# csyxwei/FFWM

Hardware: AMD Instinct MI355X
Metric: train img/s (128x128, full FFWM GAN step) (higher is better)
Workload: dtype f32; 1 GPU; BASELINE configs[2]: full FFWM train step (netG+netD+flowNetF+flowNetB, all losses, 3x Adam), synthetic MultiPIE-shaped 128x128; batch_per_gpu=8, global_batch=8, parallelism=dp1, grad_buckets=10, bucket_MiB=64

## Files before the change

### ffwm_amd/csrc/conv_winograd_gemm.hip

```cpp
#include "common.hpp"

namespace ffwm {
namespace {

typedef float f32x16 __attribute__((ext_vector_type(16)));
typedef float f32x4 __attribute__((ext_vector_type(4)));

enum { kWgNone = FFWM_WG_NONE, kWgBias = FFWM_WG_BIAS, kWgBiasRelu = FFWM_WG_BIAS_RELU, kWgBiasMfm = FFWM_WG_BIAS_MFM };
constexpr int kWgStage = 16;

struct WgGeo {
    int C, C4;
    int H, W, K;
    int TH, TW, T;
    int Tp, Kp;
};

__device__ __forceinline__ float wg_max_nan(float a, float b) { return __builtin_isunordered(a, b) ? a + b : fmaxf(a, b); }
__device__ __forceinline__ float wg_relu_nan(float v) { return v != v ? v : fmaxf(v, 0.f); }

__global__ void __launch_bounds__(kBlock)
wg_weights_kernel(const float* __restrict__ w, float* __restrict__ U, int K, int C, int Cp, int mode) {
    const int64_t e = static_cast<int64_t>(blockIdx.x) * kBlock + threadIdx.x;
    if (e >= static_cast<int64_t>(K) * Cp) return;
    const int k = static_cast<int>(e / Cp), c = static_cast<int>(e - static_cast<int64_t>(k) * Cp);
    float g[3][3];
#pragma unroll
    for (int r = 0; r < 3; ++r)
#pragma unroll
        for (int s = 0; s < 3; ++s) {
            float v = 0.f;
            if (c < C) v = mode == 0 ? w[(static_cast<size_t>(k) * C + c) * 9 + r * 3 + s]
                                     : w[(static_cast<size_t>(c) * K + k) * 9 + (2 - r) * 3 + (2 - s)];
            g[r][s] = v;
        }
    float t[4][3];
#pragma unroll
    for (int s = 0; s < 3; ++s) {
        t[0][s] = g[0][s];
        t[1][s] = 0.5f * (g[0][s] + g[1][s] + g[2][s]);
        t[2][s] = 0.5f * (g[0][s] - g[1][s] + g[2][s]);
        t[3][s] = g[2][s];
    }
    const size_t pstride = static_cast<size_t>(Cp / 4) * K * 4;
    float* dst = U + (static_cast<size_t>(c >> 2) * K + k) * 4 + (c & 3);
#pragma unroll
    for (int i = 0; i < 4; ++i) {
        dst[(i * 4 + 0) * pstride] = t[i][0];
        dst[(i * 4 + 1) * pstride] = 0.5f * (t[i][0] + t[i][1] + t[i][2]);
        dst[(i * 4 + 2) * pstride] = 0.5f * (t[i][0] - t[i][1] + t[i][2]);
        dst[(i * 4 + 3) * pstride] = t[i][2];
    }
}

__global__ void __launch_bounds__(kBlock)
wg_input_transform_kernel(const float* __restrict__ x, const float* __restrict__ mask, float* __restrict__ V, const WgGeo g) {
    const int t = blockIdx.x * kBlock + threadIdx.x;
    if (t >= g.Tp) return;
    const int c4 = blockIdx.y;
    const bool tv = t < g.T;
    const int per = g.TH * g.TW;
    const int b = tv ? t / per : 0;
    const int rem = tv ? t - b * per : 0;
    const int ty = rem / g.TW, tx = rem - ty * g.TW;
    const size_t HW = static_cast<size_t>(g.H) * g.W;
    f32x4 v[16];
#pragma unroll
    for (int j = 0; j < 4; ++j) {
        const int c = c4 * 4 + j;
        const bool cv = tv && c < g.C;
        const size_t plane = (static_cast<size_t>(b) * g.C + (cv ? c : 0)) * HW;
        float d[16];
#pragma unroll
        for (int i = 0; i < 4; ++i)
#pragma unroll
            for (int q = 0; q < 4; ++q) {
                const int iy = 2 * ty - 1 + i, ix = 2 * tx - 1 + q;
                float e = 0.f;
                if (cv && iy >= 0 && iy < g.H && ix >= 0 && ix < g.W) {
                    const size_t o = plane + static_cast<size_t>(iy) * g.W + ix;
                    e = x[o];
                    if (mask != nullptr) e = mask[o] <= 0.f ? 0.f : e;
                }
                d[i * 4 + q] = e;
            }
#pragma unroll
        for (int i = 0; i < 4; ++i) {
            float r[4];
#pragma unroll
            for (int q = 0; q < 4; ++q)
                r[q] = i == 0 ? d[0 + q] - d[8 + q] : i == 1 ? d[4 + q] + d[8 + q] : i == 2 ? d[8 + q] - d[4 + q] : d[4 + q] - d[12 + q];
            v[i * 4 + 0][j] = r[0] - r[2];
            v[i * 4 + 1][j] = r[1] + r[2];
            v[i * 4 + 2][j] = r[2] - r[1];
            v[i * 4 + 3][j] = r[1] - r[3];
        }
    }
    const size_t pstride = static_cast<size_t>(g.C4) * g.Tp;
    f32x4* dst = reinterpret_cast<f32x4*>(V) + static_cast<size_t>(c4) * g.Tp + t;
#pragma unroll
    for (int p = 0; p < 16; ++p) dst[p * pstride] = v[p];
}

template <int TILE>
__global__ void __launch_bounds__(kBlock)
wg_batched_gemm_kernel(const float* __restrict__ U, const float* __restrict__ V, float* __restrict__ M, int K, int C4, int Tp, int Kp,
                       int KT, int TTn) {
    constexpr int WT = TILE / 2, NB = WT / 32, NL = TILE / 64;
    __shared__ f32x4 As[2][4][TILE];
    __shared__ f32x4 Bs[2][4][TILE];
    const int lane = threadIdx.x & 63, wave = threadIdx.x >> 6;
    const int l31 = lane & 31, half = lane >> 5;
    const int wm = wave >> 1, wn = wave & 1;
    unsigned bid = blockIdx.x;
    const int tt = static_cast<int>(bid % static_cast<unsigned>(TTn));
    bid /= static_cast<unsigned>(TTn);
    const int kt = static_cast<int>(bid % static_cast<unsigned>(KT));
    const int p = static_cast<int>(bid / static_cast<unsigned>(KT));
    const int k0 = kt * TILE, t0 = tt * TILE;
    const f32x4* Up = reinterpret_cast<const f32x4*>(U) + static_cast<size_t>(p) * C4 * K;
    const f32x4* Vp = reinterpret_cast<const f32x4*>(V) + static_cast<size_t>(p) * C4 * Tp;

    f32x4 ra[NL], rb[NL];
    auto gload = [&](int stage) {
#pragma unroll
        for (int i = 0; i < NL; ++i) {
            const int idx = threadIdx.x + kBlock * i;
            const int grp = stage * 4 + idx / TILE, n = idx % TILE;
            f32x4 a = {0.f, 0.f, 0.f, 0.f};
            if (k0 + n < K) a = Up[static_cast<size_t>(grp) * K + k0 + n];
            ra[i] = a;
            rb[i] = Vp[static_cast<size_t>(grp) * Tp + t0 + n];
        }
    };
    auto sstore = [&](int buf) {
#pragma unroll
        for (int i = 0; i < NL; ++i) {
            const int idx = threadIdx.x + kBlock * i;
            As[buf][idx / TILE][idx % TILE] = ra[i];
            Bs[buf][idx / TILE][idx % TILE] = rb[i];
        }
    };

    f32x16 acc[NB][NB];
#pragma unroll
    for (int i = 0; i < NB; ++i)
#pragma unroll
        for (int j = 0; j < NB; ++j)
#pragma unroll
            for (int r = 0; r < 16; ++r) acc[i][j][r] = 0.f;

    const int stages = C4 / 4;
    gload(0);
    sstore(0);
    __syncthreads();
    int buf = 0;
    for (int st = 0; st < stages; ++st) {
        const bool more = st + 1 < stages;
        if (more) gload(st + 1);
#pragma unroll
        for (int s = 0; s < 2; ++s) {
            f32x4 a[NB], b[NB];
#pragma unroll
            for (int i = 0; i < NB; ++i) {
                a[i] = As[buf][2 * s + half][wm * WT + i * 32 + l31];
                b[i] = Bs[buf][2 * s + half][wn * WT + i * 32 + l31];
            }
#pragma unroll
            for (int q = 0; q < 4; ++q)
#pragma unroll
                for (int i = 0; i < NB; ++i)
#pragma unroll
                    for (int j = 0; j < NB; ++j)
                        acc[i][j] = __builtin_amdgcn_mfma_f32_32x32x2f32(a[i][q], b[j][q], acc[i][j], 0, 0, 0);
        }
        if (more) sstore(buf ^ 1);
        __syncthreads();
        buf ^= 1;
    }

    float* Mp = M + (static_cast<size_t>(p) * Kp + k0 + wm * WT) * Tp + t0 + wn * WT + l31;
#pragma unroll
    for (int i = 0; i < NB; ++i)
#pragma unroll
        for (int j = 0; j < NB; ++j)
#pragma unroll
            for (int r = 0; r < 16; ++r) {
                const int row = i * 32 + (r & 3) + 8 * (r >> 2) + 4 * half;
                Mp[static_cast<size_t>(row) * Tp + j * 32] = acc[i][j][r];
            }
}

__device__ __forceinline__ void wg_tile_of(const float* __restrict__ M, size_t pstride, float bv, float (&y)[4]) {
    float z[4][2];
#pragma unroll
    for (int i = 0; i < 4; ++i) {
        const float m0 = M[(i * 4 + 0) * pstride], m1 = M[(i * 4 + 1) * pstride], m2 = M[(i * 4 + 2) * pstride], m3 = M[(i * 4 + 3) * pstride];
        z[i][0] = (m0 + m1) + m2;
        z[i][1] = (m1 - m2) - m3;
    }
#pragma unroll
    for (int j = 0; j < 2; ++j) {
        y[j] = ((z[0][j] + z[1][j]) + z[2][j]) + bv;
        y[2 + j] = ((z[1][j] - z[2][j]) - z[3][j]) + bv;
    }
}

__global__ void __launch_bounds__(kBlock)
wg_output_transform_kernel(const float* __restrict__ M, const float* __restrict__ bias, float* __restrict__ out, const WgGeo g, int epi,
                           int vec) {
    const int t = blockIdx.x * kBlock + threadIdx.x;
    if (t >= g.T) return;
    const int ko = blockIdx.y;
    const int Kout = epi == kWgBiasMfm ? g.K / 2 : g.K;
    const size_t pstride = static_cast<size_t>(g.Kp) * g.Tp;
    const bool use_bias = bias != nullptr && epi != kWgNone;
    float y[4];
    wg_tile_of(M + static_cast<size_t>(ko) * g.Tp + t, pstride, use_bias ? bias[ko] : 0.f, y);
    if (epi == kWgBiasRelu) {
#pragma unroll
        for (int v = 0; v < 4; ++v) y[v] = wg_relu_nan(y[v]);
    } else if (epi == kWgBiasMfm) {
        float y2[4];
        wg_tile_of(M + static_cast<size_t>(ko + Kout) * g.Tp + t, pstride, use_bias ? bias[ko + Kout] : 0.f, y2);
#pragma unroll
        for (int v = 0; v < 4; ++v) y[v] = wg_max_nan(y[v], y2[v]);
    }
    const int per = g.TH * g.TW;
    const int b = t / per, rem = t - b * per;
    const int ty = rem / g.TW, tx = rem - ty * g.TW;
    const int oy = 2 * ty, ox = 2 * tx;
    const bool row1 = oy + 1 < g.H, col1 = ox + 1 < g.W;
    float* o = out + ((static_cast<size_t>(b) * Kout + ko) * g.H + oy) * g.W + ox;
    if (vec) {
        *reinterpret_cast<float2*>(o) = make_float2(y[0], y[1]);
        if (row1) *reinterpret_cast<float2*>(o + g.W) = make_float2(y[2], y[3]);
    } else {
        o[0] = y[0];
        if (col1) o[1] = y[1];
        if (row1) {
            o[g.W] = y[2];
            if (col1) o[g.W + 1] = y[3];
        }
    }
}

}
}

using namespace ffwm;

static int64_t wg_round_up(int64_t v, int64_t m) { return (v + m - 1) / m * m; }

struct WgPlan {
    int tile;
    int64_t T, Tp, Kp, Cp;
    int64_t KT, TTn;
    int64_t v_floats, m_floats;
};
static WgPlan wg_plan(int64_t B, int64_t C, int64_t H, int64_t W, int64_t K, int force_tile) {
    WgPlan p;
    p.T = B * ((H + 1) / 2) * ((W + 1) / 2);
    p.Cp = wg_round_up(C, kWgStage);
    const int64_t n128 = 16 * ((K + 127) / 128) * ((p.T + 127) / 128);
    p.tile = force_tile ? force_tile : (n128 >= device_cus() ? 128 : 64);
    p.Tp = wg_round_up(p.T, p.tile);
    p.Kp = wg_round_up(K, p.tile);
    p.KT = p.Kp / p.tile;
    p.TTn = p.Tp / p.tile;
    p.v_floats = 16 * p.Cp * p.Tp;
    p.m_floats = 16 * p.Kp * p.Tp;
    return p;
}

extern "C" int64_t ffwm_conv3x3_wg_weights_bytes(int64_t K, int64_t C) {
    if (K <= 0 || C <= 0) return 0;
    return 16 * wg_round_up(C, kWgStage) * K * 4;
}

extern "C" int64_t ffwm_conv3x3_wg_workspace_bytes(int64_t B, int64_t C, int64_t H, int64_t W, int64_t K) {
    if (B <= 0 || C <= 0 || H <= 0 || W <= 0 || K <= 0) return 0;
    const int64_t T = wg_round_up(B * ((H + 1) / 2) * ((W + 1) / 2), 128);
    return 16 * T * (wg_round_up(C, kWgStage) + wg_round_up(K, 128)) * 4;
}

extern "C" int ffwm_conv3x3_wg_weights(const void* weight, void* U, int64_t K, int64_t C, int data_gradient, int dtype, void* stream) {
    const char* fn = "ffwm_conv3x3_wg_weights";
    FFWM_REQUIRE(dtype == FFWM_F32, FFWM_ERR_DTYPE, "%s: float32 only", fn);
    FFWM_REQUIRE(weight && U, FFWM_ERR_ARG, "%s: NULL tensor pointer", fn);
    FFWM_REQUIRE(K > 0 && C > 0, FFWM_ERR_ARG, "%s: sizes must be positive", fn);
    FFWM_REQUIRE(data_gradient == 0 || data_gradient == 1, FFWM_ERR_ARG, "%s: data_gradient must be 0 or 1", fn);
    const int64_t Cp = wg_round_up(C, kWgStage);
    FFWM_REQUIRE(K * Cp < (1LL << 31) - kBlock && K * C * 9 < (1LL << 31), FFWM_ERR_SIZE, "%s: weight beyond 2^31 elements", fn);
    hipStream_t st = static_cast<hipStream_t>(stream);
    LaunchScope ls("conv_wg_weights", st, 4.0 * (9.0 * K * C + 16.0 * K * Cp));
    hipLaunchKernelGGL(wg_weights_kernel, dim3(static_cast<unsigned>((K * Cp + kBlock - 1) / kBlock)), dim3(kBlock), 0, st,
                       static_cast<const float*>(weight), static_cast<float*>(U), static_cast<int>(K), static_cast<int>(C),
                       static_cast<int>(Cp), data_gradient);
    return check_launch(fn);
}

extern "C" int ffwm_conv3x3_wg_tile(int64_t B, int64_t C, int64_t H, int64_t W, int64_t K) {
    if (B <= 0 || C <= 0 || H <= 0 || W <= 0 || K <= 0) return 0;
    return wg_plan(B, C, H, W, K, 0).tile;
}

extern "C" int ffwm_conv3x3_wg_forward(const void* input, const void* U, const void* bias, void* output, void* workspace,
                                       int64_t B, int64_t C, int64_t H, int64_t W, int64_t K, int epilogue, const void* relu_mask,
                                       int dtype, void* stream) {
    return ffwm_conv3x3_wg_forward_tiled(input, U, bias, output, workspace, B, C, H, W, K, epilogue, relu_mask, 0, dtype, stream);
}

extern "C" int ffwm_conv3x3_wg_forward_tiled(const void* input, const void* U, const void* bias, void* output, void* workspace,
                                             int64_t B, int64_t C, int64_t H, int64_t W, int64_t K, int epilogue, const void* relu_mask,
                                             int tile, int dtype, void* stream) {
    const char* fn = "ffwm_conv3x3_wg_forward";
    FFWM_REQUIRE(dtype == FFWM_F32, FFWM_ERR_DTYPE, "%s: float32 only", fn);
    FFWM_REQUIRE(input && U && output && workspace, FFWM_ERR_ARG, "%s: NULL tensor pointer", fn);
    FFWM_REQUIRE(B > 0 && C > 0 && H > 0 && W > 0 && K > 0, FFWM_ERR_ARG, "%s: sizes must be positive", fn);
    const int epi = epilogue;
    FFWM_REQUIRE(epi >= kWgNone && epi <= kWgBiasMfm, FFWM_ERR_ARG,
                 "%s: epilogue must be 0 (none), 1 (bias), 2 (bias, relu) or 3 (bias, max-feature-map)", fn);
    FFWM_REQUIRE(tile == 0 || tile == 64 || tile == 128, FFWM_ERR_ARG, "%s: tile must be 0 (the plan's), 64 or 128", fn);
    FFWM_REQUIRE(epi != kWgBiasMfm || K % 2 == 0, FFWM_ERR_ARG, "%s: the max-feature-map epilogue needs an even K", fn);
    FFWM_REQUIRE(reinterpret_cast<uintptr_t>(workspace) % 16 == 0 && reinterpret_cast<uintptr_t>(U) % 16 == 0, FFWM_ERR_ARG,
                 "%s: U and the workspace must be 16-byte aligned", fn);
    FFWM_REQUIRE(B * C * H * W < (1LL << 31) && B * K * H * W < (1LL << 31), FFWM_ERR_SIZE, "%s: a tensor beyond 2^31 elements", fn);
    const WgPlan p = wg_plan(B, C, H, W, K, tile);
    const int64_t Kout = epi == kWgBiasMfm ? K / 2 : K;
    FFWM_REQUIRE(p.Tp < (1LL << 30) && p.Cp / 4 <= 65535 && Kout <= 65535 && 16 * p.KT * p.TTn < (1LL << 31), FFWM_ERR_SIZE,
                 "%s: too many tiles or channels", fn);
    WgGeo g;
    g.C = static_cast<int>(C); g.C4 = static_cast<int>(p.Cp / 4);
    g.H = static_cast<int>(H); g.W = static_cast<int>(W); g.K = static_cast<int>(K);
    g.TH = static_cast<int>((H + 1) / 2); g.TW = static_cast<int>((W + 1) / 2); g.T = static_cast<int>(p.T);
    g.Tp = static_cast<int>(p.Tp); g.Kp = static_cast<int>(p.Kp);
    hipStream_t st = static_cast<hipStream_t>(stream);
    float* V = static_cast<float*>(workspace);
    float* M = V + p.v_floats;
    const double act = static_cast<double>(B) * H * W;
    {
        LaunchScope ls("conv_wg_in", st, 4.0 * (act * C * (relu_mask ? 2.0 : 1.0) + static_cast<double>(p.v_floats)));
        hipLaunchKernelGGL(wg_input_transform_kernel, dim3(static_cast<unsigned>((p.Tp + kBlock - 1) / kBlock), static_cast<unsigned>(g.C4)),
                           dim3(kBlock), 0, st, static_cast<const float*>(input), static_cast<const float*>(relu_mask), V, g);
    }
    if (int rc = check_launch(fn)) return rc;
    {
        LaunchScope ls("conv_wg_gemm", st, 4.0 * (16.0 * K * p.Cp + static_cast<double>(p.v_floats) + static_cast<double>(p.m_floats)),
                       2.0 * 16.0 * static_cast<double>(p.T) * K * C);
        const unsigned grid = static_cast<unsigned>(16 * p.KT * p.TTn);
        const bool ok = dispatch<64, 128>(p.tile, [&](auto TILE) {
            hipLaunchKernelGGL(wg_batched_gemm_kernel<TILE.value>, dim3(grid), dim3(kBlock), 0, st, static_cast<const float*>(U), V, M, g.K,
                               g.C4, g.Tp, g.Kp, static_cast<int>(p.KT), static_cast<int>(p.TTn));
        });
        if (!ok) return no_kernel(fn);
    }
    if (int rc = check_launch(fn)) return rc;
    {
        LaunchScope ls("conv_wg_out", st, 4.0 * (16.0 * K * p.T + act * Kout));
        const int vec = W % 2 == 0 && reinterpret_cast<uintptr_t>(output) % 8 == 0;
        hipLaunchKernelGGL(wg_output_transform_kernel, dim3(static_cast<unsigned>((p.T + kBlock - 1) / kBlock), static_cast<unsigned>(Kout)),
                           dim3(kBlock), 0, st, M, static_cast<const float*>(bias), static_cast<float*>(output), g, epi, vec);
    }
    return check_launch(fn);
}
```

Baseline: 221.4 img/s.

## Split Winograd batched GEMM reduction across waves with LDS partial-sum combine

Restructures the Winograd batched GEMM so each wave owns a fixed 64x64 output subtile, and the channel (reduction) dimension is split across KS wave groups that combine their partial sums through LDS at the end. Block size now depends on tile and split factor, which gives more waves per block for small grids. Global loads are prefetched two stages ahead using register double buffering with clamped indices instead of zero-fill branches. XCD block remapping is added for small grids. The cost is an extra LDS reduction pass and larger register and LDS footprints, which may reduce occupancy.

```diff
diff --git a/ffwm_amd/csrc/conv_winograd_gemm.hip b/ffwm_amd/csrc/conv_winograd_gemm.hip
--- a/ffwm_amd/csrc/conv_winograd_gemm.hip
+++ b/ffwm_amd/csrc/conv_winograd_gemm.hip
@@ -102,17 +102,30 @@
     for (int p = 0; p < 16; ++p) dst[p * pstride] = v[p];
 }
 
-template <int TILE>
-__global__ void __launch_bounds__(kBlock)
+template <int TILE, int KS>
+struct WgGemm {
+    static constexpr int SP = TILE / 64, SW = SP * SP;
+    static constexpr int PP = KS == 4 ? 1 : 2;
+    static constexpr int NT = SW * KS * 64;
+    static constexpr int G = 2 * KS * PP;
+    static_assert(G * 4 == kWgStage || G * 4 == 2 * kWgStage, "a stage is one or two of the 16-channel units Cp is padded to");
+};
+
+template <int TILE, int KS>
+__global__ void __launch_bounds__((WgGemm<TILE, KS>::NT))
 wg_batched_gemm_kernel(const float* __restrict__ U, const float* __restrict__ V, float* __restrict__ M, int K, int C4, int Tp, int Kp,
-                       int KT, int TTn) {
-    constexpr int WT = TILE / 2, NB = WT / 32, NL = TILE / 64;
-    __shared__ f32x4 As[2][4][TILE];
-    __shared__ f32x4 Bs[2][4][TILE];
-    const int lane = threadIdx.x & 63, wave = threadIdx.x >> 6;
+                       int KT, int TTn, int remap) {
+    using Cfg = WgGemm<TILE, KS>;
+    constexpr int SP = Cfg::SP, SW = Cfg::SW, PP = Cfg::PP, NT = Cfg::NT, G = Cfg::G;
+    constexpr int NL = G * TILE / NT;
+    static_assert(NL * NT == G * TILE, "the staging copy must divide among the threads");
+    constexpr int kStaging = 2 * 2 * G * TILE, kPartials = SW * 4 * (KS - 1) * 16 * 64 / 4;
+    __shared__ f32x4 lds[kStaging > kPartials ? kStaging : kPartials];
+    const int lane = threadIdx.x & 63, wave = __builtin_amdgcn_readfirstlane(threadIdx.x >> 6);
     const int l31 = lane & 31, half = lane >> 5;
-    const int wm = wave >> 1, wn = wave & 1;
-    unsigned bid = blockIdx.x;
+    const int sw = wave % SW, ks = wave / SW;
+    const int wm = sw / SP, wn = sw % SP;
+    unsigned bid = xcd_remap(blockIdx.x, gridDim.x, remap);
     const int tt = static_cast<int>(bid % static_cast<unsigned>(TTn));
     bid /= static_cast<unsigned>(TTn);
     const int kt = static_cast<int>(bid % static_cast<unsigned>(KT));
@@ -121,74 +134,107 @@
     const f32x4* Up = reinterpret_cast<const f32x4*>(U) + static_cast<size_t>(p) * C4 * K;
     const f32x4* Vp = reinterpret_cast<const f32x4*>(V) + static_cast<size_t>(p) * C4 * Tp;
 
-    f32x4 ra[NL], rb[NL];
-    auto gload = [&](int stage) {
+    const int stages = (C4 + G - 1) / G;
+    f32x4 ra[2][NL], rb[2][NL];
+    auto gload = [&](int stage, auto SET) {
+        constexpr int set = decltype(SET)::value;
 #pragma unroll
         for (int i = 0; i < NL; ++i) {
-            const int idx = threadIdx.x + kBlock * i;
-            const int grp = stage * 4 + idx / TILE, n = idx % TILE;
-            f32x4 a = {0.f, 0.f, 0.f, 0.f};
-            if (k0 + n < K) a = Up[static_cast<size_t>(grp) * K + k0 + n];
-            ra[i] = a;
-            rb[i] = Vp[static_cast<size_t>(grp) * Tp + t0 + n];
+            const int idx = threadIdx.x + NT * i;
+            const int grp = min(min(stage, stages - 1) * G + idx / TILE, C4 - 1), n = idx % TILE;
+            ra[set][i] = Up[static_cast<size_t>(grp) * K + min(k0 + n, K - 1)];
+            rb[set][i] = Vp[static_cast<size_t>(grp) * Tp + t0 + n];
         }
     };
-    auto sstore = [&](int buf) {
+    auto sstore = [&](int buf, auto SET) {
+        constexpr int set = decltype(SET)::value;
 #pragma unroll
         for (int i = 0; i < NL; ++i) {
-            const int idx = threadIdx.x + kBlock * i;
-            As[buf][idx / TILE][idx % TILE] = ra[i];
-            Bs[buf][idx / TILE][idx % TILE] = rb[i];
+            const int idx = threadIdx.x + NT * i;
+            lds[(buf * 2 + 0) * G * TILE + idx] = ra[set][i];
+            lds[(buf * 2 + 1) * G * TILE + idx] = rb[set][i];
         }
     };
 
-    f32x16 acc[NB][NB];
-#pragma unroll
-    for (int i = 0; i < NB; ++i)
-#pragma unroll
-        for (int j = 0; j < NB; ++j)
+    f32x16 acc[2][2];
+#pragma unroll
+    for (int i = 0; i < 2; ++i)
+#pragma unroll
+        for (int j = 0; j < 2; ++j)
 #pragma unroll
             for (int r = 0; r < 16; ++r) acc[i][j][r] = 0.f;
 
-    const int stages = C4 / 4;
-    gload(0);
-    sstore(0);
+    auto mma = [&](int buf, int pair) {
+        const f32x4* As = lds + ((buf * 2 + 0) * G + 2 * pair + half) * TILE + wm * 64 + l31;
+        const f32x4* Bs = lds + ((buf * 2 + 1) * G + 2 * pair + half) * TILE + wn * 64 + l31;
+        f32x4 a[2], b[2];
+#pragma unroll
+        for (int i = 0; i < 2; ++i) {
+            a[i] = As[i * 32];
+            b[i] = Bs[i * 32];
+        }
+#pragma unroll
+        for (int q = 0; q < 4; ++q)
+#pragma unroll
+            for (int i = 0; i < 2; ++i)
+#pragma unroll
+                for (int j = 0; j < 2; ++j) acc[i][j] = __builtin_amdgcn_mfma_f32_32x32x2f32(a[i][q], b[j][q], acc[i][j], 0, 0, 0);
+    };
+    auto step = [&](int st, auto PAR) {
+        constexpr int par = decltype(PAR)::value;
+        gload(st + 2, PAR);
+        __builtin_amdgcn_sched_barrier(0);
+#pragma unroll
+        for (int s = 0; s < PP; ++s) mma(par, s * KS + ks);
+        sstore(par ^ 1, std::integral_constant<int, (par ^ 1)>{});
+        __syncthreads();
+    };
+    const std::integral_constant<int, 0> even;
+    const std::integral_constant<int, 1> odd;
+    const int full = C4 / G;
+    gload(0, even);
+    sstore(0, even);
+    gload(1, odd);
     __syncthreads();
-    int buf = 0;
-    for (int st = 0; st < stages; ++st) {
-        const bool more = st + 1 < stages;
-        if (more) gload(st + 1);
-#pragma unroll
-        for (int s = 0; s < 2; ++s) {
-            f32x4 a[NB], b[NB];
-#pragma unroll
-            for (int i = 0; i < NB; ++i) {
-                a[i] = As[buf][2 * s + half][wm * WT + i * 32 + l31];
-                b[i] = Bs[buf][2 * s + half][wn * WT + i * 32 + l31];
-            }
-#pragma unroll
-            for (int q = 0; q < 4; ++q)
-#pragma unroll
-                for (int i = 0; i < NB; ++i)
-#pragma unroll
-                    for (int j = 0; j < NB; ++j)
-                        acc[i][j] = __builtin_amdgcn_mfma_f32_32x32x2f32(a[i][q], b[j][q], acc[i][j], 0, 0, 0);
-        }
-        if (more) sstore(buf ^ 1);
-        __syncthreads();
-        buf ^= 1;
-    }
-
-    float* Mp = M + (static_cast<size_t>(p) * Kp + k0 + wm * WT) * Tp + t0 + wn * WT + l31;
-#pragma unroll
-    for (int i = 0; i < NB; ++i)
-#pragma unroll
-        for (int j = 0; j < NB; ++j)
-#pragma unroll
-            for (int r = 0; r < 16; ++r) {
-                const int row = i * 32 + (r & 3) + 8 * (r >> 2) + 4 * half;
-                Mp[static_cast<size_t>(row) * Tp + j * 32] = acc[i][j][r];
-            }
+    for (int st = 0; st < full; st += 2) {
+        step(st, even);
+        if (st + 1 >= full) break;
+        step(st + 1, odd);
+    }
+    if (full < stages) {
+#pragma unroll
+        for (int s = 0; s < PP; ++s)
+            if (s * KS + ks < G / 4) mma(full & 1, s * KS + ks);
+    }
+    __syncthreads();
+
+    float* red = reinterpret_cast<float*>(lds);
+    constexpr int kQuad = 16 * 64;
+#pragma unroll
+    for (int q = 0; q < 4; ++q) {
+        const int own = q % KS;
+        if (ks != own) {
+            float* dst = red + static_cast<size_t>((sw * 4 + q) * (KS - 1) + (ks < own ? ks : ks - 1)) * kQuad + lane;
+#pragma unroll
+            for (int r = 0; r < 16; ++r) dst[r * 64] = acc[q >> 1][q & 1][r];
+        }
+    }
+    __syncthreads();
+    float* Mp = M + (static_cast<size_t>(p) * Kp + k0 + wm * 64) * Tp + t0 + wn * 64 + l31;
+#pragma unroll
+    for (int q = 0; q < 4; ++q) {
+        if (ks != q % KS) continue;
+        const float* src = red + static_cast<size_t>((sw * 4 + q) * (KS - 1)) * kQuad + lane;
+#pragma unroll
+        for (int o = 0; o < KS - 1; ++o)
+#pragma unroll
+            for (int r = 0; r < 16; ++r) acc[q >> 1][q & 1][r] += src[o * kQuad + r * 64];
+#pragma unroll
+        for (int r = 0; r < 16; ++r) {
+            const int row = (q >> 1) * 32 + (r & 3) + 8 * (r >> 2) + 4 * half;
+            Mp[static_cast<size_t>(row) * Tp + (q & 1) * 32] = acc[q >> 1][q & 1][r];
+        }
+    }
 }
 
 __device__ __forceinline__ void wg_tile_of(const float* __restrict__ M, size_t pstride, float bv, float (&y)[4]) {
@@ -254,6 +300,8 @@
 
 struct WgPlan {
     int tile;
+    int slices;
+    int group;
     int64_t T, Tp, Kp, Cp;
     int64_t KT, TTn;
     int64_t v_floats, m_floats;
@@ -268,6 +316,8 @@
     p.Kp = wg_round_up(K, p.tile);
     p.KT = p.Kp / p.tile;
     p.TTn = p.Tp / p.tile;
+    p.slices = p.tile == 64 ? 4 : (16 * p.KT * p.TTn <= 2 * device_cus() ? 2 : 1);
+    p.group = options().xcd_remap && 16 * p.KT * p.TTn < 2 * device_cus();
     p.v_floats = 16 * p.Cp * p.Tp;
     p.m_floats = 16 * p.Kp * p.Tp;
     return p;
@@ -350,8 +400,14 @@
                        2.0 * 16.0 * static_cast<double>(p.T) * K * C);
         const unsigned grid = static_cast<unsigned>(16 * p.KT * p.TTn);
         const bool ok = dispatch<64, 128>(p.tile, [&](auto TILE) {
-            hipLaunchKernelGGL(wg_batched_gemm_kernel<TILE.value>, dim3(grid), dim3(kBlock), 0, st, static_cast<const float*>(U), V, M, g.K,
-                               g.C4, g.Tp, g.Kp, static_cast<int>(p.KT), static_cast<int>(p.TTn));
+            auto launch = [&](auto KS) {
+                hipLaunchKernelGGL((wg_batched_gemm_kernel<TILE.value, KS.value>), dim3(grid), dim3(WgGemm<TILE.value, KS.value>::NT), 0,
+                                   st, static_cast<const float*>(U), V, M, g.K, g.C4, g.Tp, g.Kp, static_cast<int>(p.KT),
+                                   static_cast<int>(p.TTn), p.group);
+            };
+            if constexpr (TILE.value == 64) launch(std::integral_constant<int, 4>{});
+            else if (p.slices == 2) launch(std::integral_constant<int, 2>{});
+            else launch(std::integral_constant<int, 1>{});
         });
         if (!ok) return no_kernel(fn);
     }
```

Result: no change. 221.2 img/s (median of 2 runs) (-0.1%).
